# DecaYale/RSLO

Hardware: AMD Instinct MI355X
Metric: frame-pairs/sec fwd+bwd (synthetic KITTI-shaped ~122k-pt scans) (higher is better)
Workload: dtype f32; 1 GPU; C3: full fwd+bwd (voxelize + GU encoder + BEV head/vote + chamfer/ICP loss + Adam step), bs=4 frame pairs/GPU, fp32, 64-ring scans (~122412 pts/frame), dp1; frame_pairs_per_gpu=4, points_per_frame=122412, voxelize_in_step=True, voxelize_prefetch_stream=True, distinct_batches=3, optimizer_in_step=True, head_graph=fwd

## Files before the change

rslo_amd/csrc/loss.hip:

```cpp
#include <string.h>

#include <rocprim/rocprim.hpp>

#include "rslo_common.h"

#define LS_THREADS 256

struct Cov7 {
  float lam[3];
  float qn;
  float qh[4];
  float qhn;
  float qt[4];
  float V[9];
};

__device__ __forceinline__ void cov_build(const float *__restrict__ p, Cov7 &c, float S[9]) {
  c.lam[0] = p[0];
  c.lam[1] = c.lam[0] + p[1];
  c.lam[2] = c.lam[1] + p[2];
  const float n = sqrtf(p[3] * p[3] + p[4] * p[4] + p[5] * p[5] + p[6] * p[6]);
  c.qn = n;
  const float inv = 1.0f / (n + 1e-9f);
#pragma unroll
  for (int k = 0; k < 4; ++k) c.qh[k] = p[3 + k] * inv;
  float hn = sqrtf(c.qh[0] * c.qh[0] + c.qh[1] * c.qh[1] + c.qh[2] * c.qh[2] + c.qh[3] * c.qh[3]);
  hn = fmaxf(hn, 1e-12f);
  c.qhn = hn;
#pragma unroll
  for (int k = 0; k < 4; ++k) c.qt[k] = c.qh[k] / hn;
  const float x = c.qt[0], y = c.qt[1], z = c.qt[2], w = c.qt[3];
  const float tx = 2.f * x, ty = 2.f * y, tz = 2.f * z;
  const float twx = tx * w, twy = ty * w, twz = tz * w;
  const float txx = tx * x, txy = ty * x, txz = tz * x;
  const float tyy = ty * y, tyz = tz * y, tzz = tz * z;
  float *V = c.V;
  V[0] = 1.f - (tyy + tzz); V[1] = txy - twz;         V[2] = txz + twy;
  V[3] = txy + twz;         V[4] = 1.f - (txx + tzz); V[5] = tyz - twx;
  V[6] = txz - twy;         V[7] = tyz + twx;         V[8] = 1.f - (txx + tyy);
#pragma unroll
  for (int a = 0; a < 3; ++a)
#pragma unroll
    for (int b = 0; b < 3; ++b)
      S[a * 3 + b] = V[a * 3 + 0] * c.lam[0] * V[b * 3 + 0] + V[a * 3 + 1] * c.lam[1] * V[b * 3 + 1] +
                     V[a * 3 + 2] * c.lam[2] * V[b * 3 + 2];
}

__device__ __forceinline__ void cov_backward(const float *__restrict__ p, const Cov7 &c, const float G[9],
                                             float g[7]) {
  const float *V = c.V;
  float GV[9];
#pragma unroll
  for (int a = 0; a < 3; ++a)
#pragma unroll
    for (int k = 0; k < 3; ++k) GV[a * 3 + k] = G[a * 3 + 0] * V[0 * 3 + k] + G[a * 3 + 1] * V[1 * 3 + k] + G[a * 3 + 2] * V[2 * 3 + k];
  float dl[3];
#pragma unroll
  for (int k = 0; k < 3; ++k) dl[k] = V[0 * 3 + k] * GV[0 * 3 + k] + V[1 * 3 + k] * GV[1 * 3 + k] + V[2 * 3 + k] * GV[2 * 3 + k];
  g[0] = dl[0] + dl[1] + dl[2];
  g[1] = dl[1] + dl[2];
  g[2] = dl[2];
  float dV[9];
#pragma unroll
  for (int a = 0; a < 3; ++a)
#pragma unroll
    for (int k = 0; k < 3; ++k) dV[a * 3 + k] = 2.f * c.lam[k] * GV[a * 3 + k];
  const float x = c.qt[0], y = c.qt[1], z = c.qt[2], w = c.qt[3];
  float dq[4];
  dq[0] = dV[1] * 2 * y + dV[2] * 2 * z + dV[3] * 2 * y - dV[4] * 4 * x - dV[5] * 2 * w + dV[6] * 2 * z + dV[7] * 2 * w - dV[8] * 4 * x;
  dq[1] = -dV[0] * 4 * y + dV[1] * 2 * x + dV[2] * 2 * w + dV[3] * 2 * x + dV[5] * 2 * z - dV[6] * 2 * w + dV[7] * 2 * z - dV[8] * 4 * y;
  dq[2] = -dV[0] * 4 * z - dV[1] * 2 * w + dV[2] * 2 * x + dV[3] * 2 * w - dV[4] * 4 * z + dV[5] * 2 * y + dV[6] * 2 * x + dV[7] * 2 * y;
  dq[3] = -dV[1] * 2 * z + dV[2] * 2 * y + dV[3] * 2 * z - dV[5] * 2 * x - dV[6] * 2 * y + dV[7] * 2 * x;
  float dot = c.qt[0] * dq[0] + c.qt[1] * dq[1] + c.qt[2] * dq[2] + c.qt[3] * dq[3];
  float dh[4];
#pragma unroll
  for (int k = 0; k < 4; ++k) dh[k] = (dq[k] - c.qt[k] * dot) / c.qhn;
  const float n = c.qn, ne = n + 1e-9f;
  float qd = p[3] * dh[0] + p[4] * dh[1] + p[5] * dh[2] + p[6] * dh[3];
  const float coef = (n > 0.f) ? qd / (n * ne * ne) : 0.f;
#pragma unroll
  for (int k = 0; k < 4; ++k) g[3 + k] = dh[k] / ne - p[3 + k] * coef;
}

__device__ __forceinline__ float inv3(const float S[9], float I[9]) {
  const float a = S[0], b = S[1], c = S[2], d = S[3], e = S[4], f = S[5], g = S[6], h = S[7], i = S[8];
  const float A = e * i - f * h, B = -(d * i - f * g), C = d * h - e * g;
  const float det = a * A + b * B + c * C;
  const float r = 1.0f / det;
  I[0] = A * r;  I[1] = -(b * i - c * h) * r;  I[2] = (b * f - c * e) * r;
  I[3] = B * r;  I[4] = (a * i - c * g) * r;   I[5] = -(a * f - c * d) * r;
  I[6] = C * r;  I[7] = -(a * h - b * g) * r;  I[8] = (a * e - b * d) * r;
  return det;
}

__device__ __forceinline__ void sigma_of(const float S1[9], const float S2[9], const float R[9], float sg[9]) {
  float RS[9];
#pragma unroll
  for (int a = 0; a < 3; ++a)
#pragma unroll
    for (int b = 0; b < 3; ++b) RS[a * 3 + b] = R[a * 3 + 0] * S2[0 * 3 + b] + R[a * 3 + 1] * S2[1 * 3 + b] + R[a * 3 + 2] * S2[2 * 3 + b];
#pragma unroll
  for (int a = 0; a < 3; ++a)
#pragma unroll
    for (int b = 0; b < 3; ++b)
      sg[a * 3 + b] = S1[a * 3 + b] + RS[a * 3 + 0] * R[b * 3 + 0] + RS[a * 3 + 1] * R[b * 3 + 1] + RS[a * 3 + 2] * R[b * 3 + 2];
}

__device__ __forceinline__ double block_sum(double v, double *sh) {
#pragma unroll
  for (int d = 32; d >= 1; d >>= 1) v += __shfl_down(v, d, 64);
  const int lane = threadIdx.x & 63, wid = threadIdx.x >> 6;
  __syncthreads();
  if (lane == 0) sh[wid] = v;
  __syncthreads();
  double s = 0.0;
  if (threadIdx.x == 0)
    for (int w = 0; w < LS_THREADS / 64; ++w) s += sh[w];
  return s;
}

__global__ __launch_bounds__(LS_THREADS) void k_resid_fwd(const float *__restrict__ p1, const float *__restrict__ tgt,
                                                          const float *__restrict__ cov1, const float *__restrict__ cov2,
                                                          const int32_t *__restrict__ idx, const float *__restrict__ dist,
                                                          const float *__restrict__ thr, const float *__restrict__ Rd,
                                                          int N, int M, double *__restrict__ partial) {
  __shared__ double sh[LS_THREADS / 64];
  const int b = blockIdx.y;
  const int i = blockIdx.x * LS_THREADS + threadIdx.x;
  double sq = 0.0, ld = 0.0, cnt = 0.0;
  if (i < N && dist[(int64_t)b * N + i] < thr[b]) {
    const int j = idx[(int64_t)b * N + i];
    const float *a = p1 + ((int64_t)b * N + i) * 3, *t = tgt + ((int64_t)b * M + j) * 3;
    float R[9];
#pragma unroll
    for (int k = 0; k < 9; ++k) R[k] = Rd[b * 9 + k];
    Cov7 c1, c2;
    float S1[9], S2[9], sg[9], I[9];
    cov_build(cov1 + ((int64_t)b * N + i) * 7, c1, S1);
    cov_build(cov2 + ((int64_t)b * M + j) * 7, c2, S2);
    sigma_of(S1, S2, R, sg);
    const float det = inv3(sg, I);
    const float d0 = a[0] - t[0], d1 = a[1] - t[1], d2 = a[2] - t[2];
    const float v0 = I[0] * d0 + I[1] * d1 + I[2] * d2, v1 = I[3] * d0 + I[4] * d1 + I[5] * d2,
                v2 = I[6] * d0 + I[7] * d1 + I[8] * d2;
    sq = (double)(d0 * v0 + d1 * v1 + d2 * v2);
    ld = (double)(0.5f * logf(det));
    cnt = 1.0;
  }
  const double s0 = block_sum(sq, sh), s1 = block_sum(ld, sh), s2 = block_sum(cnt, sh);
  if (threadIdx.x == 0) {
    double *o = partial + ((int64_t)b * gridDim.x + blockIdx.x) * 3;
    o[0] = s0; o[1] = s1; o[2] = s2;
  }
}

__global__ void k_resid_finish(const double *__restrict__ partial, int nblk, float reg, float *__restrict__ loss,
                               float *__restrict__ cnt_out) {
  __shared__ double sh[64 * 3];
  const int b = blockIdx.x;
  double s0 = 0, s1 = 0, s2 = 0;
  for (int k0 = 0; k0 < nblk; k0 += 64) {
    const int nk = nblk - k0 < 64 ? nblk - k0 : 64;
    for (int i = threadIdx.x; i < nk * 3; i += blockDim.x) sh[i] = partial[((int64_t)b * nblk + k0) * 3 + i];
    __syncthreads();
    if (threadIdx.x == 0)
      for (int k = 0; k < nk; ++k) {
        s0 += sh[k * 3 + 0]; s1 += sh[k * 3 + 1]; s2 += sh[k * 3 + 2];
      }
    __syncthreads();
  }
  if (threadIdx.x != 0) return;
  loss[b] = (float)(s0 / s2 + (double)reg * (s1 / s2));
  cnt_out[b] = (float)s2;
}

extern "C" size_t rslo_cov_residual_ws_bytes(int B, int N) {
  return (size_t)(B > 0 ? B : 1) * (size_t)rslo_cdiv(N > 0 ? N : 1, LS_THREADS) * 3 * sizeof(double);
}

extern "C" int rslo_cov_residual_fwd(const float *p1, const float *tgt, const float *cov1, const float *cov2,
                                              const int32_t *idx, const float *dist, const float *thr,
                                              const float *Rd, int B, int N, int M, float reg_weight, void *ws,
                                              size_t ws_bytes, float *loss, float *cnt, void *stream) {
  hipStream_t st = (hipStream_t)stream;
  if (B == 0) return RSLO_OK;
  RSLO_CHECK_ARG(N >= 1 && M >= 1, "cov_residual_fwd: empty clouds");
  if (ws_bytes < rslo_cov_residual_ws_bytes(B, N)) {
    rslo_set_error("cov_residual_fwd: workspace too small");
    return RSLO_EWS;
  }
  const int nblk = (int)rslo_cdiv(N, LS_THREADS);
  hipLaunchKernelGGL(k_resid_fwd, dim3(nblk, B), dim3(LS_THREADS), 0, st, p1, tgt, cov1, cov2, idx, dist, thr, Rd, N,
                     M, (double *)ws);
  hipLaunchKernelGGL(k_resid_finish, dim3(B), dim3(64), 0, st, (const double *)ws, nblk, reg_weight, loss, cnt);
  RSLO_CHECK_LAUNCH("cov_residual_fwd");
  return RSLO_OK;
}

#define RB_THREADS 64
#define RB_NV 10
#define RB_SRC_BITS 32
#define RB_SHORT 32
__global__ __launch_bounds__(RB_THREADS) void k_resid_bwd(const float *__restrict__ p1, const float *__restrict__ tgt,
                                                          const float *__restrict__ cov1, const float *__restrict__ cov2,
                                                          const int32_t *__restrict__ idx, const float *__restrict__ dist,
                                                          const float *__restrict__ thr, const float *__restrict__ Rd,
                                                          const float *__restrict__ gloss, const float *__restrict__ cnt,
                                                          int N, int M, float reg, float *__restrict__ gp1,
                                                          float *__restrict__ gtgt, float *__restrict__ gcov1,
                                                          float *__restrict__ gcov2, float *__restrict__ contrib,
                                                          unsigned long long *__restrict__ keys, int *__restrict__ n_long) {
  const int b = blockIdx.y;
  const int i = blockIdx.x * RB_THREADS + threadIdx.x;
  const int lane = threadIdx.x;
  const bool in_range = i < N;
  if (i < M) {
    float *gt = gtgt + ((int64_t)b * M + i) * 3, *g2 = gcov2 + ((int64_t)b * M + i) * 7;
    gt[0] = gt[1] = gt[2] = 0.f;
#pragma unroll
    for (int k = 0; k < 7; ++k) g2[k] = 0.f;
  }
  if (b == 0 && i == 0) *n_long = 0;
  const bool roi = in_range && (dist[(int64_t)b * N + i] < thr[b]);
  float sc[10];
#pragma unroll
  for (int k = 0; k < 10; ++k) sc[k] = 0.f;
  int j = -1 - lane;
  if (in_range && !roi) {
    float *g1 = gcov1 + ((int64_t)b * N + i) * 7;
#pragma unroll
    for (int k = 0; k < 7; ++k) g1[k] = 0.f;
    if (gp1) {
      gp1[((int64_t)b * N + i) * 3 + 0] = 0.f;
      gp1[((int64_t)b * N + i) * 3 + 1] = 0.f;
      gp1[((int64_t)b * N + i) * 3 + 2] = 0.f;
    }
  }
  if (roi) {
    float *g1 = gcov1 + ((int64_t)b * N + i) * 7;
    const float wgt = gloss[b] / cnt[b];
    j = idx[(int64_t)b * N + i];
    const float *a = p1 + ((int64_t)b * N + i) * 3, *t = tgt + ((int64_t)b * M + j) * 3;
    const float *pc1 = cov1 + ((int64_t)b * N + i) * 7, *pc2 = cov2 + ((int64_t)b * M + j) * 7;
    float R[9];
#pragma unroll
    for (int k = 0; k < 9; ++k) R[k] = Rd[b * 9 + k];
    Cov7 c1, c2;
    float S1[9], S2[9], sg[9], I[9];
    cov_build(pc1, c1, S1);
    cov_build(pc2, c2, S2);
    sigma_of(S1, S2, R, sg);
    inv3(sg, I);
    const float d0 = a[0] - t[0], d1 = a[1] - t[1], d2 = a[2] - t[2];
    float v[3] = {I[0] * d0 + I[1] * d1 + I[2] * d2, I[3] * d0 + I[4] * d1 + I[5] * d2,
                  I[6] * d0 + I[7] * d1 + I[8] * d2};
    float G[9];
#pragma unroll
    for (int r = 0; r < 3; ++r)
#pragma unroll
      for (int c = 0; c < 3; ++c)
        G[r * 3 + c] = wgt * (-v[r] * v[c] + reg * 0.25f * (I[r * 3 + c] + I[c * 3 + r]));
    const float u0 = I[0] * d0 + I[3] * d1 + I[6] * d2, u1 = I[1] * d0 + I[4] * d1 + I[7] * d2,
                u2 = I[2] * d0 + I[5] * d1 + I[8] * d2;
    const float gd[3] = {wgt * (v[0] + u0), wgt * (v[1] + u1), wgt * (v[2] + u2)};
    if (gp1) {
      gp1[((int64_t)b * N + i) * 3 + 0] = gd[0];
      gp1[((int64_t)b * N + i) * 3 + 1] = gd[1];
      gp1[((int64_t)b * N + i) * 3 + 2] = gd[2];
    }
    sc[0] = -gd[0];
    sc[1] = -gd[1];
    sc[2] = -gd[2];
    float g7[7];
    cov_backward(pc1, c1, G, g7);
#pragma unroll
    for (int k = 0; k < 7; ++k) g1[k] = g7[k];
    float RtG[9], G2[9];
#pragma unroll
    for (int r = 0; r < 3; ++r)
#pragma unroll
      for (int c = 0; c < 3; ++c) RtG[r * 3 + c] = R[0 * 3 + r] * G[0 * 3 + c] + R[1 * 3 + r] * G[1 * 3 + c] + R[2 * 3 + r] * G[2 * 3 + c];
#pragma unroll
    for (int r = 0; r < 3; ++r)
#pragma unroll
      for (int c = 0; c < 3; ++c) G2[r * 3 + c] = RtG[r * 3 + 0] * R[0 * 3 + c] + RtG[r * 3 + 1] * R[1 * 3 + c] + RtG[r * 3 + 2] * R[2 * 3 + c];
    cov_backward(pc2, c2, G2, g7);
#pragma unroll
    for (int k = 0; k < 7; ++k) sc[3 + k] = g7[k];
  }
  if (in_range) {
    float *o = contrib + ((int64_t)b * N + i) * RB_NV;
#pragma unroll
    for (int k = 0; k < 10; ++k) o[k] = sc[k];
    keys[(int64_t)b * N + i] = roi ? ((((unsigned long long)b * M + j) << RB_SRC_BITS) | ((unsigned long long)b * N + i)) : ~0ull;
  }
}

__global__ __launch_bounds__(256) void k_resid_gather(const unsigned long long *__restrict__ skeys, int64_t n,
                                                      const float *__restrict__ contrib, float *__restrict__ gtgt,
                                                      float *__restrict__ gcov2, int *__restrict__ n_long,
                                                      int64_t *__restrict__ long_list) {
  const int64_t p = (int64_t)blockIdx.x * 256 + threadIdx.x;
  if (p >= n) return;
  const unsigned long long k = skeys[p];
  if (k == ~0ull) return;
  const unsigned long long row = k >> RB_SRC_BITS;
  if (p > 0 && (skeys[p - 1] >> RB_SRC_BITS) == row) return;
  int64_t e = p + 1;
  while (e < n && e - p <= RB_SHORT && (skeys[e] >> RB_SRC_BITS) == row) ++e;
  if (e - p > RB_SHORT) {
    long_list[atomicAdd(n_long, 1)] = p;
    return;
  }
  float acc[RB_NV];
#pragma unroll
  for (int q = 0; q < RB_NV; ++q) acc[q] = 0.f;
  for (int64_t t = p; t < e; ++t) {
    const float *c = contrib + (int64_t)(unsigned)skeys[t] * RB_NV;
#pragma unroll
    for (int q = 0; q < RB_NV; ++q) acc[q] += c[q];
  }
  float *gt = gtgt + (int64_t)row * 3, *g2 = gcov2 + (int64_t)row * 7;
  gt[0] = acc[0]; gt[1] = acc[1]; gt[2] = acc[2];
#pragma unroll
  for (int q = 0; q < 7; ++q) g2[q] = acc[3 + q];
}

__global__ __launch_bounds__(64) void k_resid_gather_long(const unsigned long long *__restrict__ skeys, int64_t n,
                                                          const float *__restrict__ contrib, float *__restrict__ gtgt,
                                                          float *__restrict__ gcov2, const int *__restrict__ n_long,
                                                          const int64_t *__restrict__ long_list) {
  const int lane = threadIdx.x;
  for (int s = blockIdx.x; s < *n_long; s += gridDim.x) {
    const int64_t p = long_list[s];
    const unsigned long long row = skeys[p] >> RB_SRC_BITS;
    float acc[RB_NV];
#pragma unroll
    for (int q = 0; q < RB_NV; ++q) acc[q] = 0.f;
    for (int64_t t = p + lane; t < n && (skeys[t] >> RB_SRC_BITS) == row; t += 64) {
      const float *c = contrib + (int64_t)(unsigned)skeys[t] * RB_NV;
#pragma unroll
      for (int q = 0; q < RB_NV; ++q) acc[q] += c[q];
    }
#pragma unroll
    for (int q = 0; q < RB_NV; ++q)
      for (int o = 32; o > 0; o >>= 1) acc[q] += __shfl_down(acc[q], o, 64);
    if (lane == 0) {
      float *gt = gtgt + (int64_t)row * 3, *g2 = gcov2 + (int64_t)row * 7;
      gt[0] = acc[0]; gt[1] = acc[1]; gt[2] = acc[2];
#pragma unroll
      for (int q = 0; q < 7; ++q) g2[q] = acc[3 + q];
    }
  }
}

static int resid_key_bits(int B, int M) {
  int bits = 1;
  while ((1ull << bits) <= (unsigned long long)B * (unsigned long long)M) ++bits;
  return bits + RB_SRC_BITS;
}

static size_t resid_sort_tmp_bytes(int64_t n, int bits) {
  size_t tmp = 0;
  (void)rocprim::radix_sort_keys(nullptr, tmp, (unsigned long long *)nullptr, (unsigned long long *)nullptr, (size_t)n,
                                 (unsigned)RB_SRC_BITS, (unsigned)bits, (hipStream_t)0);
  return (tmp + 255) / 256 * 256;
}

extern "C" size_t rslo_cov_residual_bwd_ws_bytes(int B, int N, int M) {
  if (B <= 0 || N <= 0 || M <= 0) return 256;
  const int64_t n = (int64_t)B * N;
  return (size_t)n * RB_NV * 4 + (size_t)n * 8 * 2 + (size_t)(n / RB_SHORT + 2) * 8 + 256 + resid_sort_tmp_bytes(n, resid_key_bits(B, M)) +
         8 * 256;
}

extern "C" int rslo_cov_residual_bwd(const float *p1, const float *tgt, const float *cov1, const float *cov2,
                                              const int32_t *idx, const float *dist, const float *thr,
                                              const float *Rd, const float *gloss, const float *cnt, int B, int N,
                                              int M, float reg_weight, float *gp1 , float *gtgt,
                                              float *gcov1, float *gcov2, void *ws, size_t ws_bytes, void *stream) {
  hipStream_t st = (hipStream_t)stream;
  if (B == 0) return RSLO_OK;
  const int64_t n = (int64_t)B * N;
  RSLO_CHECK_ARG(n < (1ll << 31) && (int64_t)B * M < (1ll << 31), "cov_residual_bwd: more than 2^31 rows");
  RSLO_CHECK_ARG(ws && ws_bytes >= rslo_cov_residual_bwd_ws_bytes(B, N, M), "cov_residual_bwd: workspace too small");
  const int bits = resid_key_bits(B, M);
  unsigned char *w = (unsigned char *)(((uintptr_t)ws + 255) & ~(uintptr_t)255);
  auto take = [&](size_t bytes) { unsigned char *p = w; w += (bytes + 255) / 256 * 256; return p; };
  float *contrib = (float *)take((size_t)n * RB_NV * 4);
  unsigned long long *keys = (unsigned long long *)take((size_t)n * 8);
  unsigned long long *skeys = (unsigned long long *)take((size_t)n * 8);
  int64_t *long_list = (int64_t *)take((size_t)(n / RB_SHORT + 2) * 8);
  int *n_long = (int *)take(256);
  size_t tmp = resid_sort_tmp_bytes(n, bits);
  hipLaunchKernelGGL(k_resid_bwd, dim3((unsigned)rslo_cdiv(N > M ? N : M, RB_THREADS), B), dim3(RB_THREADS), 0, st, p1, tgt,
                     cov1, cov2, idx, dist, thr, Rd, gloss, cnt, N, M, reg_weight, gp1, gtgt, gcov1, gcov2, contrib, keys,
                     n_long);
  RSLO_CHECK_LAUNCH("cov_residual_bwd");
  RSLO_HIP(rocprim::radix_sort_keys((void *)w, tmp, keys, skeys, (size_t)n, (unsigned)RB_SRC_BITS, (unsigned)bits, st));
  hipLaunchKernelGGL(k_resid_gather, dim3((unsigned)rslo_cdiv(n, 256)), dim3(256), 0, st, (const unsigned long long *)skeys, n,
                     (const float *)contrib, gtgt, gcov2, n_long, long_list);
  hipLaunchKernelGGL(k_resid_gather_long, dim3(512), dim3(64), 0, st, (const unsigned long long *)skeys, n,
                     (const float *)contrib, gtgt, gcov2, (const int *)n_long, (const int64_t *)long_list);
  RSLO_CHECK_LAUNCH("cov_residual_bwd(gather)");
  return RSLO_OK;
}

#define ICP_NM 23

__global__ __launch_bounds__(LS_THREADS) void k_icp_moments(const float *__restrict__ p1, const float *__restrict__ n1,
                                                            const float *__restrict__ tgt, const int32_t *__restrict__ idx,
                                                            const float *__restrict__ dist, const float *__restrict__ thr,
                                                            int N, int M, double *__restrict__ partial) {
  __shared__ double sh[LS_THREADS / 64];
  const int b = blockIdx.y;
  const int i = blockIdx.x * LS_THREADS + threadIdx.x;
  double mo[ICP_NM];
#pragma unroll
  for (int k = 0; k < ICP_NM; ++k) mo[k] = 0.0;
  if (i < N && dist[(int64_t)b * N + i] < thr[b]) {
    const int j = idx[(int64_t)b * N + i];
    const float *s = p1 + ((int64_t)b * N + i) * 3, *t = tgt + ((int64_t)b * M + j) * 3;
    const float *n = n1 + ((int64_t)b * N + i) * 3;
    const float e0 = t[0] - s[0], e1 = t[1] - s[1], e2 = t[2] - s[2];
    const float dot = n[0] * e0 + n[1] * e1 + n[2] * e2;
    const float nn = n[0] * n[0] + n[1] * n[1] + n[2] * n[2], ee = e0 * e0 + e1 * e1 + e2 * e2;
    const float c = dot / (fmaxf(sqrtf(nn), 1e-8f) * fmaxf(sqrtf(ee), 1e-8f));
    const double w = (double)(fabsf(c) * fabsf(c));
    mo[0] = 1.0;
    mo[7] = w;
#pragma unroll
    for (int a = 0; a < 3; ++a) {
      mo[1 + a] = s[a];
      mo[4 + a] = t[a];
      mo[8 + a] = w * s[a];
      mo[11 + a] = w * t[a];
#pragma unroll
      for (int c2 = 0; c2 < 3; ++c2) mo[14 + a * 3 + c2] = w * (double)s[a] * (double)t[c2];
    }
  }
  double *o = partial + ((int64_t)b * gridDim.x + blockIdx.x) * ICP_NM;
#pragma unroll
  for (int k = 0; k < ICP_NM; ++k) {
    const double sres = block_sum(mo[k], sh);
    if (threadIdx.x == 0) o[k] = sres;
  }
}

__device__ void svd3_jacobi(const double H[9], double U[9], double S[3], double V[9]) {
  double A[9];
  for (int k = 0; k < 9; ++k) { A[k] = H[k]; V[k] = (k % 4 == 0) ? 1.0 : 0.0; }
  for (int sweep = 0; sweep < 30; ++sweep) {
    double off = 0.0;
    for (int p = 0; p < 2; ++p)
      for (int q = p + 1; q < 3; ++q) {
        double al = 0, be = 0, ga = 0;
        for (int k = 0; k < 3; ++k) { al += A[k * 3 + p] * A[k * 3 + p]; be += A[k * 3 + q] * A[k * 3 + q]; ga += A[k * 3 + p] * A[k * 3 + q]; }
        off = fmax(off, fabs(ga) / (sqrt(al * be) + 1e-300));
        if (fabs(ga) <= 1e-300 || fabs(ga) <= 1e-17 * sqrt(al * be)) continue;
        const double zeta = (be - al) / (2.0 * ga);
        const double t = (zeta >= 0 ? 1.0 : -1.0) / (fabs(zeta) + sqrt(1.0 + zeta * zeta));
        const double c = 1.0 / sqrt(1.0 + t * t), s = c * t;
        for (int k = 0; k < 3; ++k) {
          const double ap = A[k * 3 + p], aq = A[k * 3 + q];
          A[k * 3 + p] = c * ap - s * aq;
          A[k * 3 + q] = s * ap + c * aq;
          const double vp = V[k * 3 + p], vq = V[k * 3 + q];
          V[k * 3 + p] = c * vp - s * vq;
          V[k * 3 + q] = s * vp + c * vq;
        }
      }
    if (off < 1e-15) break;
  }
  for (int k = 0; k < 3; ++k) S[k] = sqrt(A[0 * 3 + k] * A[0 * 3 + k] + A[1 * 3 + k] * A[1 * 3 + k] + A[2 * 3 + k] * A[2 * 3 + k]);
  for (int a = 0; a < 2; ++a)
    for (int b2 = a + 1; b2 < 3; ++b2)
      if (S[b2] > S[a]) {
        const double ts = S[a]; S[a] = S[b2]; S[b2] = ts;
        for (int k = 0; k < 3; ++k) {
          double tmp = A[k * 3 + a]; A[k * 3 + a] = A[k * 3 + b2]; A[k * 3 + b2] = tmp;
          tmp = V[k * 3 + a]; V[k * 3 + a] = V[k * 3 + b2]; V[k * 3 + b2] = tmp;
        }
      }
  const double tiny = 1e-14 * (S[0] > 0 ? S[0] : 1.0);
  for (int k = 0; k < 3; ++k) {
    if (S[k] > tiny) {
      for (int r = 0; r < 3; ++r) U[r * 3 + k] = A[r * 3 + k] / S[k];
    } else if (k == 2) {
      U[0 * 3 + 2] = U[1 * 3 + 0] * U[2 * 3 + 1] - U[2 * 3 + 0] * U[1 * 3 + 1];
      U[1 * 3 + 2] = U[2 * 3 + 0] * U[0 * 3 + 1] - U[0 * 3 + 0] * U[2 * 3 + 1];
      U[2 * 3 + 2] = U[0 * 3 + 0] * U[1 * 3 + 1] - U[1 * 3 + 0] * U[0 * 3 + 1];
    } else if (k == 1) {
      int ax = 0;
      for (int r = 1; r < 3; ++r)
        if (fabs(U[r * 3 + 0]) < fabs(U[ax * 3 + 0])) ax = r;
      double v[3], nn = 0.0;
      for (int r = 0; r < 3; ++r) {
        v[r] = (r == ax ? 1.0 : 0.0) - U[ax * 3 + 0] * U[r * 3 + 0];
        nn += v[r] * v[r];
      }
      for (int r = 0; r < 3; ++r) U[r * 3 + 1] = v[r] / sqrt(nn);
    } else {
      for (int r = 0; r < 3; ++r) U[r * 3 + k] = (r == k) ? 1.0 : 0.0;
    }
  }
}

__device__ double det3(const double M[9]) {
  return M[0] * (M[4] * M[8] - M[5] * M[7]) - M[1] * (M[3] * M[8] - M[5] * M[6]) + M[2] * (M[3] * M[7] - M[4] * M[6]);
}

__global__ void k_icp_solve(const double *__restrict__ partial, int nblk, float *__restrict__ res_r,
                            float *__restrict__ res_t, float *__restrict__ step_R, float *__restrict__ step_t,
                            int first) {
  const int b = blockIdx.x;
  __shared__ double mo[ICP_NM];
  for (int m = threadIdx.x >> 6; m < ICP_NM; m += blockDim.x >> 6) {
    double s = 0.0;
    for (int k = threadIdx.x & 63; k < nblk; k += 64) s += partial[((int64_t)b * nblk + k) * ICP_NM + m];
    for (int o = 32; o > 0; o >>= 1) s += __shfl_down(s, o, 64);
    if ((threadIdx.x & 63) == 0) mo[m] = s;
  }
  __syncthreads();
  if (threadIdx.x != 0) return;
  const double cnt = mo[0] > 1.0 ? mo[0] : 1.0;
  double cs[3], ct[3];
  for (int a = 0; a < 3; ++a) { cs[a] = mo[1 + a] / cnt; ct[a] = mo[4 + a] / cnt; }
  double H[9];
  for (int a = 0; a < 3; ++a)
    for (int c = 0; c < 3; ++c)
      H[a * 3 + c] = mo[14 + a * 3 + c] - mo[8 + a] * ct[c] - cs[a] * mo[11 + c] + mo[7] * cs[a] * ct[c];
  double U[9], S[3], V[9];
  svd3_jacobi(H, U, S, V);
  double VUt[9];
  for (int a = 0; a < 3; ++a)
    for (int c = 0; c < 3; ++c) VUt[a * 3 + c] = V[a * 3 + 0] * U[c * 3 + 0] + V[a * 3 + 1] * U[c * 3 + 1] + V[a * 3 + 2] * U[c * 3 + 2];
  double R[9];
  if (det3(VUt) < 0.0) {
    for (int a = 0; a < 3; ++a)
      for (int c = 0; c < 3; ++c) R[a * 3 + c] = V[a * 3 + 0] * U[c * 3 + 0] + V[a * 3 + 1] * U[c * 3 + 1] - V[a * 3 + 2] * U[c * 3 + 2];
  } else {
    for (int k = 0; k < 9; ++k) R[k] = VUt[k];
  }
  double t[3], Ri[9], ti[3];
  for (int a = 0; a < 3; ++a) t[a] = -(R[a * 3 + 0] * cs[0] + R[a * 3 + 1] * cs[1] + R[a * 3 + 2] * cs[2]) + ct[a];
  for (int a = 0; a < 3; ++a)
    for (int c = 0; c < 3; ++c) Ri[a * 3 + c] = R[c * 3 + a];
  for (int a = 0; a < 3; ++a) ti[a] = -(Ri[a * 3 + 0] * t[0] + Ri[a * 3 + 1] * t[1] + Ri[a * 3 + 2] * t[2]);
  if (step_R)
    for (int k = 0; k < 9; ++k) step_R[b * 9 + k] = (float)Ri[k];
  if (step_t)
    for (int a = 0; a < 3; ++a) step_t[b * 3 + a] = (float)ti[a];
  double rr[9], rt[3];
  for (int k = 0; k < 9; ++k) rr[k] = first ? (k % 4 == 0 ? 1.0 : 0.0) : (double)res_r[b * 9 + k];
  for (int a = 0; a < 3; ++a) rt[a] = first ? 0.0 : (double)res_t[b * 3 + a];
  for (int a = 0; a < 3; ++a) {
    for (int c = 0; c < 3; ++c)
      res_r[b * 9 + a * 3 + c] = (float)(Ri[a * 3 + 0] * rr[0 * 3 + c] + Ri[a * 3 + 1] * rr[1 * 3 + c] + Ri[a * 3 + 2] * rr[2 * 3 + c]);
    res_t[b * 3 + a] = (float)(Ri[a * 3 + 0] * rt[0] + Ri[a * 3 + 1] * rt[1] + Ri[a * 3 + 2] * rt[2] + ti[a]);
  }
}

extern "C" size_t rslo_icp_ws_bytes(int B, int N) {
  return (size_t)(B > 0 ? B : 1) * (size_t)rslo_cdiv(N > 0 ? N : 1, LS_THREADS) * ICP_NM * sizeof(double);
}

static int icp_step_launch(const float *p1, const float *n1, const float *tgt, const int32_t *idx, const float *dist,
                           const float *thr, int B, int N, int M, void *ws, size_t ws_bytes, float *res_r, float *res_t,
                           float *step_R, float *step_t, int first, void *stream) {
  hipStream_t st = (hipStream_t)stream;
  if (B == 0) return RSLO_OK;
  RSLO_CHECK_ARG(N >= 1 && M >= 1, "icp_step: empty clouds");
  if (ws_bytes < rslo_icp_ws_bytes(B, N)) {
    rslo_set_error("icp_step: workspace too small");
    return RSLO_EWS;
  }
  const int nblk = (int)rslo_cdiv(N, LS_THREADS);
  hipLaunchKernelGGL(k_icp_moments, dim3(nblk, B), dim3(LS_THREADS), 0, st, p1, n1, tgt, idx, dist, thr, N, M,
                     (double *)ws);
  hipLaunchKernelGGL(k_icp_solve, dim3(B), dim3(256), 0, st, (const double *)ws, nblk, res_r, res_t, step_R, step_t,
                     first);
  RSLO_CHECK_LAUNCH("icp_step");
  return RSLO_OK;
}

extern "C" int rslo_icp_step(const float *p1, const float *n1, const float *tgt, const int32_t *idx,
                                      const float *dist, const float *thr, int B, int N, int M, void *ws,
                                      size_t ws_bytes, float *res_r , float *res_t ,
                                      float *step_R , float *step_t , void *stream) {
  return icp_step_launch(p1, n1, tgt, idx, dist, thr, B, N, M, ws, ws_bytes, res_r, res_t, step_R, step_t, 0, stream);
}

extern "C" int rslo_icp_step_first(const float *p1, const float *n1, const float *tgt, const int32_t *idx,
                                   const float *dist, const float *thr, int B, int N, int M, void *ws, size_t ws_bytes,
                                   float *res_r , float *res_t , float *step_R, float *step_t,
                                   void *stream) {
  return icp_step_launch(p1, n1, tgt, idx, dist, thr, B, N, M, ws, ws_bytes, res_r, res_t, step_R, step_t, 1, stream);
}

__global__ void k_transform(const float *__restrict__ x, const float *__restrict__ R, const float *__restrict__ t, int M,
                            float *__restrict__ out) {
  const int b = blockIdx.y;
  const int j = blockIdx.x * blockDim.x + threadIdx.x;
  if (j >= M) return;
  const float *p = x + ((int64_t)b * M + j) * 3;
  const float *r = R + b * 9;
  float *o = out + ((int64_t)b * M + j) * 3;
#pragma unroll
  for (int a = 0; a < 3; ++a) o[a] = r[a * 3 + 0] * p[0] + r[a * 3 + 1] * p[1] + r[a * 3 + 2] * p[2] + t[b * 3 + a];
}

extern "C" int rslo_transform_points(const float *x, const float *R, const float *t, int B, int M, float *out,
                                              void *stream) {
  if (B == 0 || M == 0) return RSLO_OK;
  hipLaunchKernelGGL(k_transform, dim3((unsigned)rslo_cdiv(M, 256), B), dim3(256), 0, (hipStream_t)stream, x, R, t, M,
                     out);
  RSLO_CHECK_LAUNCH("transform_points");
  return RSLO_OK;
}

__device__ __forceinline__ void roi_hist_add(unsigned *hist, bool on, unsigned bin) {
  unsigned long long act = __ballot(on);
#pragma unroll
  for (int r = 0; r < 2; ++r) {
    if (act == 0ull) break;
    const int lead = __ffsll((long long)act) - 1;
    const unsigned b0 = (unsigned)__shfl((int)bin, lead);
    const bool same = on && bin == b0;
    const unsigned long long m = __ballot(same);
    if ((int)(threadIdx.x & 63u) == lead) atomicAdd(&hist[b0], (unsigned)__popcll(m));
    on = on && !same;
    act &= ~m;
  }
  if (on) atomicAdd(&hist[bin], 1u);
}

__global__ __launch_bounds__(1024) void k_roi_threshold(const float *__restrict__ dist, int N,
                                                        const int32_t *__restrict__ counts, double ratio,
                                                        float *__restrict__ thr) {
  __shared__ unsigned hist[256];
  __shared__ unsigned s_prefix, s_k;
  const int b = blockIdx.x;
  const int cnt = counts ? counts[b] : N;
  const unsigned *d = reinterpret_cast<const unsigned *>(dist) + (int64_t)b * N;
  if (cnt <= 0) {
    if (threadIdx.x == 0) thr[b] = 1.0f;
    return;
  }
  long long k = 1 + (long long)((double)cnt * ratio);
  k = k > cnt ? cnt : (k < 1 ? 1 : k);
  if (threadIdx.x == 0) {
    s_prefix = 0u;
    s_k = (unsigned)k;
  }
  constexpr int ROI_RV = 40;
  unsigned vals[ROI_RV];
#pragma unroll
  for (int j = 0; j < ROI_RV; ++j) {
    const int i = (int)threadIdx.x + j * 1024;
    vals[j] = d[i < cnt ? i : cnt - 1];
  }
  for (int pass = 0; pass < 4; ++pass) {
    const int shift = 24 - 8 * pass;
    if (threadIdx.x < 256) hist[threadIdx.x] = 0u;
    __syncthreads();
    const unsigned prefix = s_prefix;
    const unsigned himask = pass == 0 ? 0u : (0xffffffffu << (shift + 8));
#pragma unroll
    for (int j = 0; j < ROI_RV; ++j) {
      const unsigned v = vals[j];
      if (j * 1024 < cnt)
        roi_hist_add(hist, (int)threadIdx.x + j * 1024 < cnt && (v & himask) == prefix, (v >> shift) & 0xffu);
    }
    for (int i0 = ROI_RV * 1024; i0 < cnt; i0 += 1024) {
      const int i = i0 + (int)threadIdx.x;
      const unsigned v = d[i < cnt ? i : cnt - 1];
      roi_hist_add(hist, i < cnt && (v & himask) == prefix, (v >> shift) & 0xffu);
    }
    __syncthreads();
    if (threadIdx.x < 64) {
      const int l = (int)threadIdx.x;
      const unsigned kk = s_k;
      unsigned h[4];
#pragma unroll
      for (int j = 0; j < 4; ++j) h[j] = hist[4 * l + j];
      const unsigned sum = h[0] + h[1] + h[2] + h[3];
      unsigned inc = sum;
#pragma unroll
      for (int o = 1; o < 64; o <<= 1) {
        const unsigned t = (unsigned)__shfl_up((int)inc, o);
        if (l >= o) inc += t;
      }
      const unsigned exc = inc - sum;
      const bool mine = exc < kk && kk <= inc;
      const unsigned long long any = __ballot(mine);
      if (mine) {
        unsigned acc = exc;
        int j = 0;
        while (j < 3 && acc + h[j] < kk) acc += h[j++];
        s_k = kk - acc;
        s_prefix = prefix | ((unsigned)(4 * l + j) << shift);
      } else if (any == 0ull && l == 63) {
        s_k = kk - inc;
        s_prefix = prefix | (255u << shift);
      }
    }
// ... 358 lines not shown
```

Baseline: 376.7 frame-pairs/s.

## Replace radix sort in residual backward with counting-sort CSR gather

The rocprim 64-bit radix sort used to group source points by target row in the covariance-residual backward is replaced with a counting sort. Per-row counts are gathered with wave-aggregated atomics, turned into offsets by a two-pass scan, and used to scatter source ids into a CSR list. Short runs are sorted per thread in shared memory, and long runs are ranked with a shared-memory bitmap, so the deterministic summation order is preserved. This removes the multi-pass sort over 8-byte keys and the zero-fill of the gradient outputs. In exchange it adds several kernel launches, a memset and atomic contention on popular rows.

```diff
diff --git a/rslo_amd/csrc/loss.hip b/rslo_amd/csrc/loss.hip
--- a/rslo_amd/csrc/loss.hip
+++ b/rslo_amd/csrc/loss.hip
@@ -1,6 +1,4 @@
 #include <string.h>
-
-#include <rocprim/rocprim.hpp>
 
 #include "rslo_common.h"
 
@@ -199,33 +197,53 @@
 
 #define RB_THREADS 64
 #define RB_NV 10
-#define RB_SRC_BITS 32
 #define RB_SHORT 32
+#define RB_PEEL 8
+#define RB_SCAN_CHUNK 1024
+#define RB_LONG_THREADS 512
+#define RB_WINDOW 65536
+
+__device__ __forceinline__ int resid_row_take(int *counter, bool on, int row) {
+  const int lane = (int)(threadIdx.x & 63u);
+  unsigned long long act = __ballot(on);
+  int add = 0, from = lane, rank = 0;
+#pragma unroll 1
+  for (int r = 0; r < RB_PEEL; ++r) {
+    if (act == 0ull) break;
+    const int lead = __ffsll((long long)act) - 1;
+    const int r0 = __shfl(row, lead);
+    const bool same = on && row == r0;
+    const unsigned long long m = __ballot(same);
+    if (lane == lead) add = __popcll(m);
+    if (same) {
+      from = lead;
+      rank = __popcll(m & ((1ull << lane) - 1ull));
+    }
+    on = on && !same;
+    act &= ~m;
+  }
+  if (on) add = 1;
+  int base = 0;
+  if (add) base = atomicAdd(&counter[row], add);
+  return __shfl(base, from) + rank;
+}
+
 __global__ __launch_bounds__(RB_THREADS) void k_resid_bwd(const float *__restrict__ p1, const float *__restrict__ tgt,
                                                           const float *__restrict__ cov1, const float *__restrict__ cov2,
                                                           const int32_t *__restrict__ idx, const float *__restrict__ dist,
                                                           const float *__restrict__ thr, const float *__restrict__ Rd,
                                                           const float *__restrict__ gloss, const float *__restrict__ cnt,
                                                           int N, int M, float reg, float *__restrict__ gp1,
-                                                          float *__restrict__ gtgt, float *__restrict__ gcov1,
-                                                          float *__restrict__ gcov2, float *__restrict__ contrib,
-                                                          unsigned long long *__restrict__ keys, int *__restrict__ n_long) {
+                                                          float *__restrict__ gcov1, float *__restrict__ contrib,
+                                                          int *__restrict__ count) {
   const int b = blockIdx.y;
   const int i = blockIdx.x * RB_THREADS + threadIdx.x;
-  const int lane = threadIdx.x;
   const bool in_range = i < N;
-  if (i < M) {
-    float *gt = gtgt + ((int64_t)b * M + i) * 3, *g2 = gcov2 + ((int64_t)b * M + i) * 7;
-    gt[0] = gt[1] = gt[2] = 0.f;
-#pragma unroll
-    for (int k = 0; k < 7; ++k) g2[k] = 0.f;
-  }
-  if (b == 0 && i == 0) *n_long = 0;
   const bool roi = in_range && (dist[(int64_t)b * N + i] < thr[b]);
   float sc[10];
 #pragma unroll
   for (int k = 0; k < 10; ++k) sc[k] = 0.f;
-  int j = -1 - lane;
+  int j = 0;
   if (in_range && !roi) {
     float *g1 = gcov1 + ((int64_t)b * N + i) * 7;
 #pragma unroll
@@ -292,86 +310,226 @@
     float *o = contrib + ((int64_t)b * N + i) * RB_NV;
 #pragma unroll
     for (int k = 0; k < 10; ++k) o[k] = sc[k];
-    keys[(int64_t)b * N + i] = roi ? ((((unsigned long long)b * M + j) << RB_SRC_BITS) | ((unsigned long long)b * N + i)) : ~0ull;
-  }
-}
-
-__global__ __launch_bounds__(256) void k_resid_gather(const unsigned long long *__restrict__ skeys, int64_t n,
+  }
+  (void)resid_row_take(count, roi, b * M + j);
+}
+
+__global__ __launch_bounds__(256) void k_resid_chunk_sums(const int *__restrict__ count, int n, int *__restrict__ sums) {
+  __shared__ int red[4];
+  const int base = blockIdx.x * RB_SCAN_CHUNK;
+  int s = 0;
+#pragma unroll
+  for (int q = 0; q < RB_SCAN_CHUNK / 256; ++q) {
+    const int r = base + q * 256 + (int)threadIdx.x;
+    s += r < n ? count[r] : 0;
+  }
+  for (int d = 32; d > 0; d >>= 1) s += __shfl_down(s, d, 64);
+  if ((threadIdx.x & 63) == 0) red[threadIdx.x >> 6] = s;
+  __syncthreads();
+  if (threadIdx.x == 0) sums[blockIdx.x] = red[0] + red[1] + red[2] + red[3];
+}
+
+__global__ __launch_bounds__(256) void k_resid_scan(int *__restrict__ count, int n, const int *__restrict__ sums) {
+  __shared__ int wsum[4];
+  __shared__ int carry_s;
+  int c = 0;
+  for (int k = threadIdx.x; k < (int)blockIdx.x; k += 256) c += sums[k];
+  for (int d = 32; d > 0; d >>= 1) c += __shfl_down(c, d, 64);
+  if ((threadIdx.x & 63) == 0) wsum[threadIdx.x >> 6] = c;
+  __syncthreads();
+  if (threadIdx.x == 0) carry_s = wsum[0] + wsum[1] + wsum[2] + wsum[3];
+  __syncthreads();
+  const int r = blockIdx.x * RB_SCAN_CHUNK + (int)threadIdx.x * 4;
+  int v[4];
+#pragma unroll
+  for (int q = 0; q < 4; ++q) v[q] = r + q < n ? count[r + q] : 0;
+  const int tot = v[0] + v[1] + v[2] + v[3];
+  int inc = tot;
+  const int lane = threadIdx.x & 63;
+  for (int d = 1; d < 64; d <<= 1) {
+    const int t = __shfl_up(inc, d, 64);
+    if (lane >= d) inc += t;
+  }
+  __syncthreads();
+  if (lane == 63) wsum[threadIdx.x >> 6] = inc;
+  __syncthreads();
+  int run = carry_s + inc - tot;
+  for (int w = 0; w < (int)(threadIdx.x >> 6); ++w) run += wsum[w];
+#pragma unroll
+  for (int q = 0; q < 4; ++q) {
+    if (r + q < n) count[r + q] = run;
+    run += v[q];
+  }
+}
+
+__global__ __launch_bounds__(256) void k_resid_place(const int32_t *__restrict__ idx, const float *__restrict__ dist,
+                                                     const float *__restrict__ thr, int N, int M, int n,
+                                                     int *__restrict__ off, int *__restrict__ list) {
+  const int p = blockIdx.x * 256 + (int)threadIdx.x;
+  const int b = p < n ? p / N : 0;
+  const bool roi = p < n && (dist[p] < thr[b]);
+  const int row = roi ? b * M + idx[p] : 0;
+  const int slot = resid_row_take(off, roi, row);
+  if (roi) list[slot] = p;
+}
+
+__device__ __forceinline__ int resid_run_start(const int *__restrict__ off, int row) { return row ? off[row - 1] : 0; }
+
+__device__ __forceinline__ void resid_row_load(const float *__restrict__ contrib, int src, float v[RB_NV]) {
+  const float2 *c = reinterpret_cast<const float2 *>(contrib + (int64_t)src * RB_NV);
+#pragma unroll
+  for (int q = 0; q < RB_NV / 2; ++q) {
+    const float2 t = c[q];
+    v[2 * q] = t.x;
+    v[2 * q + 1] = t.y;
+  }
+}
+
+__device__ __forceinline__ void resid_row_store(const float acc[RB_NV], int row, float *__restrict__ gtgt,
+                                                float *__restrict__ gcov2) {
+  float *gt = gtgt + (int64_t)row * 3, *g2 = gcov2 + (int64_t)row * 7;
+  gt[0] = acc[0]; gt[1] = acc[1]; gt[2] = acc[2];
+#pragma unroll
+  for (int q = 0; q < 7; ++q) g2[q] = acc[3 + q];
+}
+
+__global__ __launch_bounds__(256) void k_resid_gather(const int *__restrict__ off, const int *__restrict__ list, int nrows,
                                                       const float *__restrict__ contrib, float *__restrict__ gtgt,
                                                       float *__restrict__ gcov2, int *__restrict__ n_long,
-                                                      int64_t *__restrict__ long_list) {
-  const int64_t p = (int64_t)blockIdx.x * 256 + threadIdx.x;
-  if (p >= n) return;
-  const unsigned long long k = skeys[p];
-  if (k == ~0ull) return;
-  const unsigned long long row = k >> RB_SRC_BITS;
-  if (p > 0 && (skeys[p - 1] >> RB_SRC_BITS) == row) return;
-  int64_t e = p + 1;
-  while (e < n && e - p <= RB_SHORT && (skeys[e] >> RB_SRC_BITS) == row) ++e;
-  if (e - p > RB_SHORT) {
-    long_list[atomicAdd(n_long, 1)] = p;
+                                                      int *__restrict__ long_list) {
+  __shared__ int ids[RB_SHORT * 256];
+  const int row = blockIdx.x * 256 + (int)threadIdx.x;
+  if (row >= nrows) return;
+  const int s = resid_run_start(off, row), e = off[row];
+  if (e - s > RB_SHORT) {
+    long_list[atomicAdd(n_long, 1)] = row;
     return;
   }
+  const int L = e - s;
+  int *mine = ids + threadIdx.x;
+  for (int c = 0; c < L; ++c) {
+    const int v = list[s + c];
+    int k = c;
+    for (; k > 0; --k) {
+      const int w = mine[(k - 1) * 256];
+      if (w < v) break;
+      mine[k * 256] = w;
+    }
+    mine[k * 256] = v;
+  }
   float acc[RB_NV];
 #pragma unroll
   for (int q = 0; q < RB_NV; ++q) acc[q] = 0.f;
-  for (int64_t t = p; t < e; ++t) {
-    const float *c = contrib + (int64_t)(unsigned)skeys[t] * RB_NV;
-#pragma unroll
-    for (int q = 0; q < RB_NV; ++q) acc[q] += c[q];
-  }
-  float *gt = gtgt + (int64_t)row * 3, *g2 = gcov2 + (int64_t)row * 7;
-  gt[0] = acc[0]; gt[1] = acc[1]; gt[2] = acc[2];
-#pragma unroll
-  for (int q = 0; q < 7; ++q) g2[q] = acc[3 + q];
-}
-
-__global__ __launch_bounds__(64) void k_resid_gather_long(const unsigned long long *__restrict__ skeys, int64_t n,
-                                                          const float *__restrict__ contrib, float *__restrict__ gtgt,
-                                                          float *__restrict__ gcov2, const int *__restrict__ n_long,
-                                                          const int64_t *__restrict__ long_list) {
-  const int lane = threadIdx.x;
-  for (int s = blockIdx.x; s < *n_long; s += gridDim.x) {
-    const int64_t p = long_list[s];
-    const unsigned long long row = skeys[p] >> RB_SRC_BITS;
-    float acc[RB_NV];
-#pragma unroll
-    for (int q = 0; q < RB_NV; ++q) acc[q] = 0.f;
-    for (int64_t t = p + lane; t < n && (skeys[t] >> RB_SRC_BITS) == row; t += 64) {
-      const float *c = contrib + (int64_t)(unsigned)skeys[t] * RB_NV;
-#pragma unroll
-      for (int q = 0; q < RB_NV; ++q) acc[q] += c[q];
-    }
-#pragma unroll
-    for (int q = 0; q < RB_NV; ++q)
-      for (int o = 32; o > 0; o >>= 1) acc[q] += __shfl_down(acc[q], o, 64);
-    if (lane == 0) {
-      float *gt = gtgt + (int64_t)row * 3, *g2 = gcov2 + (int64_t)row * 7;
-      gt[0] = acc[0]; gt[1] = acc[1]; gt[2] = acc[2];
-#pragma unroll
-      for (int q = 0; q < 7; ++q) g2[q] = acc[3 + q];
-    }
-  }
-}
-
-static int resid_key_bits(int B, int M) {
-  int bits = 1;
-  while ((1ull << bits) <= (unsigned long long)B * (unsigned long long)M) ++bits;
-  return bits + RB_SRC_BITS;
-}
-
-static size_t resid_sort_tmp_bytes(int64_t n, int bits) {
-  size_t tmp = 0;
-  (void)rocprim::radix_sort_keys(nullptr, tmp, (unsigned long long *)nullptr, (unsigned long long *)nullptr, (size_t)n,
-                                 (unsigned)RB_SRC_BITS, (unsigned)bits, (hipStream_t)0);
-  return (tmp + 255) / 256 * 256;
+  int c = 0;
+  for (; c + 3 < L; c += 4) {
+    float v[4][RB_NV];
+#pragma unroll
+    for (int u = 0; u < 4; ++u) resid_row_load(contrib, mine[(c + u) * 256], v[u]);
+#pragma unroll
+    for (int u = 0; u < 4; ++u)
+#pragma unroll
+      for (int q = 0; q < RB_NV; ++q) acc[q] += v[u][q];
+  }
+  for (; c < L; ++c) {
+    float v[RB_NV];
+    resid_row_load(contrib, mine[c * 256], v);
+#pragma unroll
+    for (int q = 0; q < RB_NV; ++q) acc[q] += v[q];
+  }
+  resid_row_store(acc, row, gtgt, gcov2);
+}
+
+__global__ __launch_bounds__(RB_LONG_THREADS) void k_resid_gather_long(const int *__restrict__ off, const int *__restrict__ list,
+                                                                       int *ranked, int N, int M,
+                                                                       const float *__restrict__ contrib,
+                                                                       float *__restrict__ gtgt, float *__restrict__ gcov2,
+                                                                       const int *__restrict__ n_long,
+                                                                       const int *__restrict__ long_list) {
+  constexpr int WORDS = RB_WINDOW / 32, OWN = WORDS / RB_LONG_THREADS;
+  static_assert(OWN * RB_LONG_THREADS * 32 == RB_WINDOW, "RB_WINDOW: a multiple of 32 RB_LONG_THREADS");
+  __shared__ unsigned bitmap[WORDS];
+  __shared__ int below[WORDS];
+  __shared__ int wsum[RB_LONG_THREADS / 64];
+  const int tid = threadIdx.x, lane = threadIdx.x & 63, wave = threadIdx.x >> 6;
+  const int nl = *n_long;
+  for (int s = blockIdx.x; s < nl; s += gridDim.x) {
+    const int row = long_list[s];
+    const int start = resid_run_start(off, row), L = off[row] - start;
+    const int first = (row / M) * N;
+    int placed = 0;
+    for (unsigned w0 = 0; w0 < (unsigned)N && placed < L; w0 += RB_WINDOW) {
+      for (int t = tid; t < WORDS; t += RB_LONG_THREADS) bitmap[t] = 0u;
+      __syncthreads();
+      for (int t = tid; t < L; t += RB_LONG_THREADS) {
+        const unsigned i = (unsigned)(list[start + t] - first) - w0;
+        if (i < (unsigned)RB_WINDOW) atomicOr(&bitmap[i >> 5], 1u << (i & 31u));
+      }
+      __syncthreads();
+      int mine[OWN], tot = 0;
+#pragma unroll
+      for (int q = 0; q < OWN; ++q) tot += (mine[q] = __popc(bitmap[tid * OWN + q]));
+      int inc = tot;
+      for (int d = 1; d < 64; d <<= 1) {
+        const int t = __shfl_up(inc, d, 64);
+        if (lane >= d) inc += t;
+      }
+      if (lane == 63) wsum[wave] = inc;
+      __syncthreads();
+      int run = inc - tot, total = 0;
+#pragma unroll
+      for (int w = 0; w < RB_LONG_THREADS / 64; ++w) {
+        if (w < wave) run += wsum[w];
+        total += wsum[w];
+      }
+#pragma unroll
+      for (int q = 0; q < OWN; ++q) {
+        below[tid * OWN + q] = run;
+        run += mine[q];
+      }
+      __syncthreads();
+      for (int t = tid; t < L; t += RB_LONG_THREADS) {
+        const int id = list[start + t];
+        const unsigned i = (unsigned)(id - first) - w0;
+        if (i < (unsigned)RB_WINDOW)
+          ranked[start + placed + below[i >> 5] + __popc(bitmap[i >> 5] & ((1u << (i & 31u)) - 1u))] = id;
+      }
+      placed += total;
+      __syncthreads();
+    }
+    if (tid < 64) {
+      const int *run = ranked + start;
+      float acc[RB_NV];
+#pragma unroll
+      for (int q = 0; q < RB_NV; ++q) acc[q] = 0.f;
+      int t = lane;
+      for (; t + 192 < L; t += 256) {
+        float v[4][RB_NV];
+#pragma unroll
+        for (int u = 0; u < 4; ++u) resid_row_load(contrib, run[t + 64 * u], v[u]);
+#pragma unroll
+        for (int u = 0; u < 4; ++u)
+#pragma unroll
+          for (int q = 0; q < RB_NV; ++q) acc[q] += v[u][q];
+      }
+      for (; t < L; t += 64) {
+        float v[RB_NV];
+        resid_row_load(contrib, run[t], v);
+#pragma unroll
+        for (int q = 0; q < RB_NV; ++q) acc[q] += v[q];
+      }
+#pragma unroll
+      for (int q = 0; q < RB_NV; ++q)
+        for (int o = 32; o > 0; o >>= 1) acc[q] += __shfl_down(acc[q], o, 64);
+      if (lane == 0) resid_row_store(acc, row, gtgt, gcov2);
+    }
+  }
 }
 
 extern "C" size_t rslo_cov_residual_bwd_ws_bytes(int B, int N, int M) {
   if (B <= 0 || N <= 0 || M <= 0) return 256;
-  const int64_t n = (int64_t)B * N;
-  return (size_t)n * RB_NV * 4 + (size_t)n * 8 * 2 + (size_t)(n / RB_SHORT + 2) * 8 + 256 + resid_sort_tmp_bytes(n, resid_key_bits(B, M)) +
-         8 * 256;
+  const int64_t n = (int64_t)B * N, nrows = (int64_t)B * M;
+  return (size_t)n * RB_NV * 4 + (size_t)nrows * 4 + 256 + (size_t)rslo_cdiv(nrows, RB_SCAN_CHUNK) * 4 + (size_t)n * 4 * 2 +
+         (size_t)(n / RB_SHORT + 2) * 4 + 8 * 256;
 }
 
 extern "C" int rslo_cov_residual_bwd(const float *p1, const float *tgt, const float *cov1, const float *cov2,
@@ -384,24 +542,28 @@
   const int64_t n = (int64_t)B * N;
   RSLO_CHECK_ARG(n < (1ll << 31) && (int64_t)B * M < (1ll << 31), "cov_residual_bwd: more than 2^31 rows");
   RSLO_CHECK_ARG(ws && ws_bytes >= rslo_cov_residual_bwd_ws_bytes(B, N, M), "cov_residual_bwd: workspace too small");
-  const int bits = resid_key_bits(B, M);
+  const int nrows = B * M, nchunk = (int)rslo_cdiv(nrows, RB_SCAN_CHUNK);
   unsigned char *w = (unsigned char *)(((uintptr_t)ws + 255) & ~(uintptr_t)255);
   auto take = [&](size_t bytes) { unsigned char *p = w; w += (bytes + 255) / 256 * 256; return p; };
   float *contrib = (float *)take((size_t)n * RB_NV * 4);
-  unsigned long long *keys = (unsigned long long *)take((size_t)n * 8);
-  unsigned long long *skeys = (unsigned long long *)take((size_t)n * 8);
-  int64_t *long_list = (int64_t *)take((size_t)(n / RB_SHORT + 2) * 8);
+  int *off = (int *)take((size_t)nrows * 4);
   int *n_long = (int *)take(256);
-  size_t tmp = resid_sort_tmp_bytes(n, bits);
-  hipLaunchKernelGGL(k_resid_bwd, dim3((unsigned)rslo_cdiv(N > M ? N : M, RB_THREADS), B), dim3(RB_THREADS), 0, st, p1, tgt,
-                     cov1, cov2, idx, dist, thr, Rd, gloss, cnt, N, M, reg_weight, gp1, gtgt, gcov1, gcov2, contrib, keys,
-                     n_long);
+  int *sums = (int *)take((size_t)nchunk * 4);
+  int *list = (int *)take((size_t)n * 4);
+  int *ranked = (int *)take((size_t)n * 4);
+  int *long_list = (int *)take((size_t)(n / RB_SHORT + 2) * 4);
+  RSLO_HIP(hipMemsetAsync(off, 0, (size_t)((unsigned char *)n_long - (unsigned char *)off) + 256, st));
+  hipLaunchKernelGGL(k_resid_bwd, dim3((unsigned)rslo_cdiv(N, RB_THREADS), B), dim3(RB_THREADS), 0, st, p1, tgt, cov1, cov2,
+                     idx, dist, thr, Rd, gloss, cnt, N, M, reg_weight, gp1, gcov1, contrib, off);
   RSLO_CHECK_LAUNCH("cov_residual_bwd");
-  RSLO_HIP(rocprim::radix_sort_keys((void *)w, tmp, keys, skeys, (size_t)n, (unsigned)RB_SRC_BITS, (unsigned)bits, st));
-  hipLaunchKernelGGL(k_resid_gather, dim3((unsigned)rslo_cdiv(n, 256)), dim3(256), 0, st, (const unsigned long long *)skeys, n,
-                     (const float *)contrib, gtgt, gcov2, n_long, long_list);
-  hipLaunchKernelGGL(k_resid_gather_long, dim3(512), dim3(64), 0, st, (const unsigned long long *)skeys, n,
-                     (const float *)contrib, gtgt, gcov2, (const int *)n_long, (const int64_t *)long_list);
+  hipLaunchKernelGGL(k_resid_chunk_sums, dim3(nchunk), dim3(256), 0, st, (const int *)off, nrows, sums);
+  hipLaunchKernelGGL(k_resid_scan, dim3(nchunk), dim3(256), 0, st, off, nrows, (const int *)sums);
+  hipLaunchKernelGGL(k_resid_place, dim3((unsigned)rslo_cdiv(n, 256)), dim3(256), 0, st, idx, dist, thr, N, M, (int)n, off, list);
+  RSLO_CHECK_LAUNCH("cov_residual_bwd(lists)");
+  hipLaunchKernelGGL(k_resid_gather, dim3((unsigned)rslo_cdiv(nrows, 256)), dim3(256), 0, st, (const int *)off, (const int *)list,
+                     nrows, (const float *)contrib, gtgt, gcov2, n_long, long_list);
+  hipLaunchKernelGGL(k_resid_gather_long, dim3(512), dim3(RB_LONG_THREADS), 0, st, (const int *)off, (const int *)list, ranked, N, M,
+                     (const float *)contrib, gtgt, gcov2, (const int *)n_long, (const int *)long_list);
   RSLO_CHECK_LAUNCH("cov_residual_bwd(gather)");
   return RSLO_OK;
 }
```

Result: slower. 372.1 frame-pairs/s (-1.2%).
